# MarbleHE/ABC

Hardware: AMD Instinct MI355X
Metric: homomorphic mul+relin/sec, CKKS N=2^14 (higher is better)
Workload: dtype u64 (transforms: exact integer arithmetic in f64); 1 GPU; CKKS N=16384, 4 data limbs {50,40,40,40} + special 50-bit prime, ct x ct multiply + relinearize; total_batch=8192, batch_rank0=8192

## Files before the change

### abc_amd/csrc/abc_context.hip

```cpp
#include <cstdlib>
#include <cstring>
#include <mutex>

#include "../../include/abc_hip.h"
#include <dlfcn.h>

#include "abc_context.hpp"
#include "abc_host_math.hpp"

namespace abc {

static thread_local std::string g_err;
void set_error(const std::string &msg) { g_err = msg; }

static bool env_on(const char *name) {
  const char *e = std::getenv(name);
  return e && !(e[0] == '0' && e[1] == 0);
}
void read_switches(abc_hip_ctx *c) {
  abc_hip_ctx::Switches s;
  s.no_fused = env_on("ABC_HIP_NO_FUSED");
  s.no_split = env_on("ABC_HIP_NO_SPLIT");
  s.no_split4 = env_on("ABC_HIP_NO_SPLIT4");
  s.no_isplit = env_on("ABC_HIP_NO_ISPLIT");
  s.no_gsplit = env_on("ABC_HIP_NO_GSPLIT");
  s.no_bsplit = env_on("ABC_HIP_NO_BSPLIT");
  s.no_mixed = env_on("ABC_HIP_NO_MIXED");
  s.no_pack = env_on("ABC_HIP_NO_PACK");
  s.no_key_twin = env_on("ABC_HIP_NO_KEY_TWIN");
  s.no_bmul = env_on("ABC_HIP_NO_BMUL");
  s.no_special8x2 = env_on("ABC_HIP_NO_SPECIAL8X2");
  s.no_bmul_mid = env_on("ABC_HIP_NO_BMUL_MID");
  s.no_finish_lds = env_on("ABC_HIP_NO_FINISH_LDS");
  s.no_iks = env_on("ABC_HIP_NO_IKS");
  s.no_bmul_r6 = env_on("ABC_HIP_NO_BMUL_R6");
  s.no_lean_front = env_on("ABC_HIP_NO_LEAN_FRONT");
  s.no_tensor_intt = env_on("ABC_HIP_NO_TENSOR_INTT");
  s.no_galois_fusion = env_on("ABC_HIP_NO_GALOIS_FUSION");
  if (const char *e = std::getenv("ABC_HIP_CHUNK")) s.chunk = (size_t)std::atol(e);
  if (const char *e = std::getenv("ABC_HIP_FEW_LIMBS")) s.few_limbs = (size_t)std::atol(e);
  if (const char *e = std::getenv("ABC_HIP_LEAN_LIMIT")) s.lean_limit = (size_t)std::atol(e);
  if (const char *e = std::getenv("ABC_HIP_PASS0_TARGET_LIMIT")) s.pass0_target_limit = (size_t)std::atol(e);
  if (const char *e = std::getenv("ABC_HIP_BFV_SCRATCH_MB")) s.bfv_scratch_mb = (size_t)std::atol(e);
  if (const char *e = std::getenv("ABC_HIP_LANE_OFFSET_US")) s.lane_offset_us = (unsigned)std::atoi(e);
  if (const char *e = std::getenv("ABC_HIP_LANES")) {
    s.lanes = std::atoi(e);
    if (s.lanes < 1) s.lanes = 1;
    if (s.lanes > abc_hip_ctx::kMaxLanes) s.lanes = abc_hip_ctx::kMaxLanes;
  }
  c->sw = s;
}

static bool capturing(abc_hip_ctx *c) {
  hipStreamCaptureStatus st = hipStreamCaptureStatusNone;
  if (hipStreamIsCapturing(c->stream, &st) != hipSuccess) return false;
  return st != hipStreamCaptureStatusNone;
// ... 1091 lines not shown
```

### abc_amd/csrc/abc_context.hpp

```cpp
#pragma once

#include <hip/hip_runtime.h>

#include <map>
#include <mutex>
#include <unordered_map>
#include <string>
#include <vector>

#include "abc_modarith.hpp"
#include "abc_ntt.hpp"

namespace abc {

constexpr int kMaxLimbs = 16;

struct LimbMap {
  int id[kMaxLimbs + 1];
};

struct DevConst {
  u64 inv_special[kMaxLimbs], inv_special_s[kMaxLimbs];
  u64 inv_qlast[kMaxLimbs][kMaxLimbs], inv_qlast_s[kMaxLimbs][kMaxLimbs];
  u64 special_mod_q[kMaxLimbs], special_mod_q_s[kMaxLimbs];
// ... 73 lines not shown
}

struct abc_hip_ctx {
  int scheme = 0, logn = 0, n = 0, K = 0, L = 0, device = 0;
  std::vector<uint64_t> primes;
  uint64_t t = 0;
  hipStream_t stream = nullptr;
  hipStream_t own_stream = nullptr;
  hipEvent_t ev0 = nullptr, ev1 = nullptr;
  static constexpr int kMaxLanes = 4;
  hipStream_t lane[kMaxLanes] = {nullptr, nullptr, nullptr, nullptr};
  hipEvent_t lane_fork = nullptr, lane_join[kMaxLanes] = {nullptr, nullptr, nullptr, nullptr};
  std::vector<abc::Mod> h_mods;
  std::vector<uint64_t> mod_values;
  int nB = 0, nBsk = 0;
  abc::DevCtx dc{};
  abc::DevConst h_cst{};
  abc::Mod *d_mods = nullptr;
  uint64_t *d_tw = nullptr;
  double *d_ftw = nullptr;
  bool cache_alloc = false;
  std::mutex alloc_mu;
  size_t cached_bytes = 0, cache_cap = (size_t)8 << 30;
  std::unordered_map<size_t, std::vector<void *>> free_blocks;
  std::unordered_map<void *, size_t> block_size;
  bool capture_active = false;
  std::unordered_map<void *, std::vector<void *>> pin;
  std::unordered_map<void *, bool> parked;
  std::unordered_map<size_t, std::vector<void *>> cap_free;
  std::unordered_map<void *, bool> cap_born;
  bool behz_fp = false;
  bool use_fp = true;
  struct Switches {
    bool no_fused = false, no_split = false, no_split4 = false, no_isplit = false, no_gsplit = false, no_lean_front = false, no_bsplit = false, no_mixed = false, no_pack = false, no_key_twin = false, no_special8x2 = false, no_bmul = false, no_bmul_mid = false, no_finish_lds = false, no_iks = false, no_bmul_r6 = false, no_tensor_intt = false;
    bool no_galois_fusion = false;
    size_t chunk = 0, few_limbs = 48, lean_limit = 96, bfv_scratch_mb = 0, pass0_target_limit = 128;
    int lanes = 2;
    unsigned lane_offset_us = 0;
  } sw;
  abc::DevConst *d_cst = nullptr;
  abc::DevConstFp *d_cstf = nullptr;
  uint32_t *d_slot_map = nullptr;
  void *d_ckks_codec = nullptr;
  uint64_t *d_sk = nullptr, *d_pk = nullptr, *d_relin = nullptr;
  std::map<uint32_t, uint64_t *> d_galois;
  std::unordered_map<const uint64_t *, double *> key_twins;
  std::unordered_map<const uint64_t *, uint64_t *> key_shoups;
  std::vector<uint32_t> galois_order;
  void *ws = nullptr;
  size_t ws_bytes = 0;
  void *aux[3] = {nullptr, nullptr, nullptr};
  size_t aux_bytes[3] = {0, 0, 0};
  size_t limb_words() const { return (size_t)n; }
  size_t key_words() const { return (size_t)L * 2 * K * n; }
};

namespace abc {

void set_error(const std::string &msg);
#define ABC_HIP_CHECK(expr)                                                                         \
  do {                                                                                              \
    hipError_t e_ = (expr);                                                                         \
    if (e_ != hipSuccess) {                                                                         \
      abc::set_error(std::string(#expr) + ": " + hipGetErrorString(e_));                            \
      return 1;                                                                                     \
    }                                                                                               \
  } while (0)
// ... 107 lines not shown
```

### abc_amd/csrc/abc_kernels_fused.hip

```cpp
#include <type_traits>

#include "abc_context.hpp"
#include "abc_host_math.hpp"

namespace abc {

static inline unsigned stream_grid(size_t items, int block) {
  size_t g = (items + block - 1) / block;
  const size_t cap = 256 * 8 * 4;
  return (unsigned)(g < cap ? (g ? g : 1) : cap);
}

template <int LB>
__global__ __launch_bounds__((1 << LB) / 16) void k_fused_tensor_intt(DevCtx c, const u64 *__restrict__ a,
                                                                      const u64 *__restrict__ b, u64 *__restrict__ c01,
                                                                      u64 *__restrict__ c2coef, u64 *__restrict__ c2ntt, int nl) {
  __shared__ u64 lds[lds_words(LB)];
  const int j = blockIdx.x % nl;
  const size_t ct = blockIdx.x / nl;
  const size_t N = (size_t)1 << LB, pw = (size_t)nl * N;
  const Mod m = c.mods[j];
  const NttTable t = ntt_table(c, j);
  const u64 *__restrict__ a0 = a + ct * 2 * pw + j * N, *__restrict__ a1 = a0 + pw;
  const u64 *__restrict__ b0 = b + ct * 2 * pw + j * N, *__restrict__ b1 = b0 + pw;
// ... 788 lines not shown
    r.x = fp_to_canon(fp_mul_lazy(s1[0] - u1.x, inv, inv_q, q) + d1[0], q, qinv);
    r.y = fp_to_canon(fp_mul_lazy(s1[1] - u1.y, inv, inv_q, q) + d1[1], q, qinv);
    *reinterpret_cast<u64x2 *>(out + ((ct * 2 + 1) * nl + I) * N + base + e) = r;
  }
}

template <int MODE, bool GAL>
static void launch_split3_main(hipStream_t st, abc_hip_ctx *c, size_t cc, int nl, const double *part, const double *tpart, const u64 *opa,
                               const u64 *opb, size_t opa_stride, size_t opb_stride, int add_c1, const u64 *key, u64 *out, u32 gelt) {
  const dim3 grid((unsigned)(cc * nl * 16)), block(64 * (nl + 1));
  const size_t lds = (size_t)((nl + 1) * lds_words(10)) * 8;
#define ABC_TM3(NLV)                                                                                                                 \
  hipLaunchKernelGGL((k_split3_main_fp<MODE, GAL, NLV>), grid, block, lds, st, c->dc, part, tpart, opa, opb, opa_stride, opb_stride, \
                     add_c1, key, out, nl, gelt)
  switch (nl) {
    case 1: ABC_TM3(1); break;
    case 2: ABC_TM3(2); break;
    case 3: ABC_TM3(3); break;
    case 4: ABC_TM3(4); break;
    default: ABC_TM3(0); break;
  }
#undef ABC_TM3
}


template <int MODE, int NL>
struct PairOps {
  u64x2 k0[NL], k1[NL];
  u64x2 a0, a1, b0, b1;
  u64 xs[2], d0s[2], d1s[2];
};

template <int MODE, bool GAL, int NL>
__global__ __launch_bounds__(512, NL <= 4 ? 4 : 2) void k_split4_main_fp(DevCtx c, const double *__restrict__ part,
                                                                   const double *__restrict__ tpart, const u64 *__restrict__ opa,
                                                                   const u64 *__restrict__ opb, size_t opa_stride, size_t opb_stride,
                                                                   int add_c1, const u64 *__restrict__ key, u64 *__restrict__ out, u32 gelt,
                                                                   u32 imap, int ni, int pack, const double *__restrict__ keyf) {
  extern __shared__ double dyn[];
  static_assert(NL + 1 <= 8, "one wavefront per limb, eight wavefronts");
  constexpr int nl = NL, NT = 512, PER = 2;
  const int W = __builtin_amdgcn_readfirstlane((int)(threadIdx.x >> 6));
  const int lane = threadIdx.x & 63;
  const int blk = blockIdx.x & 15;
  const int I = (int)((imap >> (4 * ((blockIdx.x >> 4) % (unsigned)ni))) & 15u);
  const size_t ct = (size_t)((blockIdx.x >> 4) / (unsigned)ni);
  const size_t N = (size_t)c.n, base = (size_t)blk << 10;
  const Mod m = mod_at(c, I);
  const FpTable t = fp_table(c, I);
  const double q = m.qd, qinv = m.qinv;
  f64x2 *ltw = reinterpret_cast<f64x2 *>(dyn + (nl + 1) * lds_words(10));
  const size_t pw = (size_t)nl * N;
  const ABC_CONST_AS DevConst *cst = (const ABC_CONST_AS DevConst *)c.cst;
  const double inv = cst->inv_special_c[I], inv_q = cst->inv_special_cq[I];

  f64x2 twv[PER];
  block_twiddles_fetch<10, f64x2, PER>(t.tw, 4, blk, (int)threadIdx.x, NT, twv);
  const bool has_limb = W <= nl;
  const int Wc = has_limb ? W : 0;
  const double *__restrict__ src = (Wc < nl - 1) ? part + ((ct * (nl + 1) + I) * nl + (Wc < I ? Wc : Wc + 1)) * (size_t)c.ps + base
                                                 : tpart + ((ct * 2 + (Wc - (nl - 1))) * nl + I) * (size_t)c.ps + base;
  const int pk = pack ? pack_kind(m.bits) : 0;
  u64x2 raw[8];
  if (has_limb) {
    if (pk == 0) {
#pragma unroll
      for (int k = 0; k < 8; k++) raw[k] = *reinterpret_cast<const u64x2 *>(src + (k << 7) + 2 * lane);
    } else if (pk == 1) {
#pragma unroll
      for (int k = 0; k < 8; k++) raw[k] = pack_load_pair<1>(src - base, N, base + (k << 7) + 2 * lane);
    } else {
#pragma unroll
      for (int k = 0; k < 8; k++) raw[k] = pack_load_pair<2>(src - base, N, base + (k << 7) + 2 * lane);
    }
  }
  auto load_pair = [&](int e, PairOps<MODE, NL> &o) {
    const u64 *kw = keyf ? reinterpret_cast<const u64 *>(keyf) : key;
#pragma unroll
    for (int Jx = 0; Jx < NL; Jx++) {
      o.k0[Jx] = *reinterpret_cast<const u64x2 *>(kw + (((size_t)Jx * 2 + 0) * c.K + I) * N + base + e);
      o.k1[Jx] = *reinterpret_cast<const u64x2 *>(kw + (((size_t)Jx * 2 + 1) * c.K + I) * N + base + e);
    }
    if (MODE == 0) {
      const u64 *pa = opa + ct * 2 * pw + (size_t)I * N + base + e, *pb = opb + ct * 2 * pw + (size_t)I * N + base + e;
      o.a0 = *reinterpret_cast<const u64x2 *>(pa); o.a1 = *reinterpret_cast<const u64x2 *>(pa + pw);
      o.b0 = *reinterpret_cast<const u64x2 *>(pb); o.b1 = *reinterpret_cast<const u64x2 *>(pb + pw);
    } else {
      const u64 *xl = opa + ct * opa_stride + (size_t)I * N;
#pragma unroll
      for (int k = 0; k < 2; k++) {
        const u32 si = galois_ntt_src<GAL>((u32)(base + e + k), gelt, c.logn);
        o.xs[k] = xl[si];
        o.d0s[k] = o.d1s[k] = 0;
        if (opb) {
          const u64 *ad = opb + ct * opb_stride + (size_t)I * N;
          o.d0s[k] = ad[si];
          if (add_c1) o.d1s[k] = ad[pw + si];
        }
      }
    }
  };
  PairOps<MODE, NL> ops;
  load_pair(2 * (int)threadIdx.x, ops);

  block_twiddles_store<10, f64x2, PER>(ltw, (int)threadIdx.x, NT, twv);
  __syncthreads();
  if (has_limb) {
    double *buf = dyn + W * lds_words(10);
    double xin[16];
    if (pk == 0) {
#pragma unroll
      for (int k = 0; k < 8; k++) {
        xin[k] = __longlong_as_double((long long)raw[k].x);
        xin[8 + k] = __longlong_as_double((long long)raw[k].y);
      }
    } else if (pk == 1) {
#pragma unroll
      for (int k = 0; k < 8; k++) pack_decode_pair<1>(raw[k], xin[k], xin[8 + k]);
    } else {
#pragma unroll
      for (int k = 0; k < 8; k++) pack_decode_pair<2>(raw[k], xin[k], xin[8 + k]);
    }
    if (m.bits >= 49) {
#pragma unroll
      for (int r = 0; r < 16; r++) xin[r] = fp_centre(xin[r], q, qinv);
    }
    ntt_fwd_tail1024_pairs<FpTail>(buf, xin, [&](int, int i, double v) { buf[lds_pad(i)] = v; }, t, m, 4, blk, lane, ltw);
  }
  __syncthreads();
  const double *tt0 = dyn + (nl - 1) * lds_words(10), *tt1 = dyn + nl * lds_words(10);
  auto compute_pair = [&](int e, const PairOps<MODE, NL> &o, auto twin) {
    constexpr bool TW = decltype(twin)::value;
    auto kd = [](u64 w) { return TW ? __longlong_as_double((long long)w) : fp_from_u64(w); };
    double s0[2] = {0.0, 0.0}, s1[2] = {0.0, 0.0}, d0[2] = {0.0, 0.0}, d1[2] = {0.0, 0.0};
#pragma unroll
    for (int Jx = 0; Jx < NL; Jx++) {
      double x[2];
      if (Jx == I) {
        if (MODE == 0) {
          const double x0[2] = {fp_from_u64(o.a0.x), fp_from_u64(o.a0.y)}, x1[2] = {fp_from_u64(o.a1.x), fp_from_u64(o.a1.y)};
          const double y0[2] = {fp_from_u64(o.b0.x), fp_from_u64(o.b0.y)}, y1[2] = {fp_from_u64(o.b1.x), fp_from_u64(o.b1.y)};
#pragma unroll
          for (int k = 0; k < 2; k++) {
            x[k] = fp_mulmod(x1[k], y1[k], q, qinv);
            d0[k] = fp_mulmod(x0[k], y0[k], q, qinv);
            d1[k] = fp_mulmod(x0[k], y1[k], q, qinv) + fp_mulmod(x1[k], y0[k], q, qinv);
          }
        } else {
#pragma unroll
          for (int k = 0; k < 2; k++) {
            x[k] = fp_from_u64(o.xs[k]);
            d0[k] = fp_from_u64(o.d0s[k]);
            d1[k] = fp_from_u64(o.d1s[k]);
          }
        }
      } else {
        const int w = Jx < I ? Jx : Jx - 1;
        const f64x2 v = *reinterpret_cast<const f64x2 *>(dyn + w * lds_words(10) + lds_pad(e));
        x[0] = v.x;
        x[1] = v.y;
      }
      s0[0] += fp_mulmod(x[0], kd(o.k0[Jx].x), q, qinv);
      s0[1] += fp_mulmod(x[1], kd(o.k0[Jx].y), q, qinv);
      s1[0] += fp_mulmod(x[0], kd(o.k1[Jx].x), q, qinv);
      s1[1] += fp_mulmod(x[1], kd(o.k1[Jx].y), q, qinv);
      if (Jx == 7) {
#pragma unroll
        for (int k = 0; k < 2; k++) {
          s0[k] = fp_centre(s0[k], q, qinv);
          s1[k] = fp_centre(s1[k], q, qinv);
        }
      }
    }
    const f64x2 u0 = *reinterpret_cast<const f64x2 *>(tt0 + lds_pad(e)), u1 = *reinterpret_cast<const f64x2 *>(tt1 + lds_pad(e));
    u64x2 r;
    r.x = fp_to_canon(fp_mul_lazy(s0[0] - u0.x, inv, inv_q, q) + d0[0], q, qinv);
    r.y = fp_to_canon(fp_mul_lazy(s0[1] - u0.y, inv, inv_q, q) + d0[1], q, qinv);
    *reinterpret_cast<u64x2 *>(out + ((ct * 2 + 0) * nl + I) * N + base + e) = r;
    r.x = fp_to_canon(fp_mul_lazy(s1[0] - u1.x, inv, inv_q, q) + d1[0], q, qinv);
    r.y = fp_to_canon(fp_mul_lazy(s1[1] - u1.y, inv, inv_q, q) + d1[1], q, qinv);
    *reinterpret_cast<u64x2 *>(out + ((ct * 2 + 1) * nl + I) * N + base + e) = r;
  };
  if (keyf) compute_pair(2 * (int)threadIdx.x, ops, std::true_type{});
  else compute_pair(2 * (int)threadIdx.x, ops, std::false_type{});
}

template <int MODE, bool GAL>
static bool launch_split4_main(hipStream_t st, abc_hip_ctx *c, size_t cc, int nl, const double *part, const double *tpart, const u64 *opa,
                               const u64 *opb, size_t opa_stride, size_t opb_stride, int add_c1, const u64 *key, u64 *out, u32 gelt,
                               u32 imap = 0x76543210u, int ni = -1, int pack = 0) {
  if (nl < 1 || nl > 7) return false;
  if (ni < 0) ni = nl;
  if (ni == 0) return true;
  const dim3 grid((unsigned)(cc * ni * 16)), block(512);
  const size_t lds = (size_t)((nl + 1) * lds_words(10)) * 8 + 1024 * 16;
#define ABC_TM4(NLV)                                                                                                                 \
  hipLaunchKernelGGL((k_split4_main_fp<MODE, GAL, NLV>), grid, block, lds, st, c->dc, part, tpart, opa, opb, opa_stride, opb_stride, \
                     add_c1, key, out, gelt, imap, ni, pack, keyf)
  const double *keyf = key_twin_lookup(c, key);
  switch (nl) {
    case 1: ABC_TM4(1); break;
    case 2: ABC_TM4(2); break;
    case 3: ABC_TM4(3); break;
    case 4: ABC_TM4(4); break;
    case 5: ABC_TM4(5); break;
    case 6: ABC_TM4(6); break;
    default: ABC_TM4(7); break;
  }
#undef ABC_TM4
  return true;
}
bool split4_main_subset(hipStream_t st, abc_hip_ctx *c, size_t cc, int nl, int mode, const double *part, const double *tpart, const u64 *opa,
                        const u64 *opb, size_t opa_stride, size_t opb_stride, int add_c1, const u64 *key, u64 *out, u32 gelt, u32 imap,
                        int ni) {
  if (mode == 0) return launch_split4_main<0, false>(st, c, cc, nl, part, tpart, opa, opb, opa_stride, opb_stride, add_c1, key, out, gelt, imap, ni);
  if (gelt) return launch_split4_main<1, true>(st, c, cc, nl, part, tpart, opa, opb, opa_stride, opb_stride, add_c1, key, out, gelt, imap, ni);
  return launch_split4_main<1, false>(st, c, cc, nl, part, tpart, opa, opb, opa_stride, opb_stride, add_c1, key, out, gelt, imap, ni);
}


template <int MODE, bool GAL>
static void launch_split3(hipStream_t st, abc_hip_ctx *c, const FusedScratch &s, size_t cc, int nl, const u64 *opa, const u64 *opb,
                          size_t opa_stride, size_t opb_stride, int add_c1, const u64 *key, u64 *out, u32 gelt, int pack) {
  launch_split_special(st, c, cc, nl, (const double *)s.dec, key, (double *)s.tsp);
  hipLaunchKernelGGL(k_split3_pass_fp<14>, dim3((unsigned)(cc * 2 * 4)), dim3(256), 0, st, c->dc, (const double *)s.tsp, (double *)s.ksacc,
                     nl, pack);
  if (!c->sw.no_split4 && nl <= 5 && launch_split4_main<MODE, GAL>(st, c, cc, nl, (const double *)s.dec, (const double *)s.ksacc, opa, opb,
                                                        opa_stride, opb_stride, add_c1, key, out, gelt, 0x76543210u, -1, pack))
    return;
  launch_split3_main<MODE, GAL>(st, c, cc, nl, (const double *)s.dec, (const double *)s.ksacc, opa, opb, opa_stride, opb_stride, add_c1,
                                key, out, gelt);
}

static inline int pack_half_done(const abc_hip_ctx *c, int nl) {
  return (!c->sw.no_pack && !c->sw.no_split4 && nl >= 1 && nl <= 5) ? 1 : 0;
}
static inline bool all_fp(const abc_hip_ctx *c) {
  bool fp = c->use_fp;
  for (int j = 0; j < c->K; j++) fp = fp && fp_ok(c->h_mods[j].bits);
  return fp;
}
static inline bool needs_guard(const abc_hip_ctx *c) {
  bool guard = false;
  for (int j = 0; j < c->K; j++) guard = guard || !unguarded_ok(c->h_mods[j].bits);
  return guard;
}

template <int LB>
static int keyswitch_stage(abc_hip_ctx *c, hipStream_t st, const FusedScratch &s, const u64 *coef, size_t coef_stride, const u64 *ntt,
                           size_t ntt_stride, const u64 *key, const u64 *addend, size_t addend_stride, bool add_c1, u64 *out, int nl,
                           size_t cc, int dec_ready = 0 ) {
  const size_t N = (size_t)1 << LB;
  const dim3 block((1 << LB) / 16);
  const bool ckks = (c->scheme == 2);
  const bool guard = needs_guard(c);
  const unsigned g2a = (unsigned)(cc * (nl + 1) * nl);
  const unsigned g3 = (unsigned)(cc * 2 * nl);
  if (all_fp(c)) {
    if (!dec_ready)
// ... 330 lines not shown
```

### abc_amd/csrc/abc_ntt.hpp

```cpp
#pragma once

#include "abc_modarith.hpp"

namespace abc {

__device__ __forceinline__ int lds_pad(int i) { return i + ((i >> 6) << 2); }
constexpr int lds_words(int lb) { return (1 << lb) + ((1 << lb) >> 6) * 4; }

struct NttTable {
  const u64x2 *tw;
  const u64x2 *itw;
};
struct alignas(16) f64x2 {
  double x, y;
};
#define ABC_CONST_AS __attribute__((address_space(4)))
struct FpTable {
  const ABC_CONST_AS f64x2 *tw, *itw;
};
__device__ __forceinline__ f64x2 tw_load(const ABC_CONST_AS f64x2 *p) {
  f64x2 r;
  r.x = p->x;
  r.y = p->y;
  return r;
// ... 115 lines not shown
    if (PASS > 0 && k.red) centre16(x, k);
  }
  template <int PASS> __device__ __forceinline__ static void inv_begin(E (&x)[16], const K &k) {
    if (PASS > 0 || k.red) centre16(x, k);
  }
};

struct FpTail : FpArith {
  template <int PASS> __device__ __forceinline__ static void fwd_begin(E (&x)[16], const K &k) {
    if (PASS == 2 && k.red && k.q >= 562949953421312.0) centre16(x, k);
  }
};

template <class A, int LB, int S, int R>
__device__ __forceinline__ void fwd_pass(typename A::E (&x)[16], const int (&hi)[16 >> R], const typename A::Table &t,
                                         const typename A::K &kk, int S0, int b) {
  constexpr int NG = 16 >> R;
#pragma unroll
  for (int u = 0; u < R; u++) {
    const int half = 1 << (R - 1 - u);
#pragma unroll
    for (int g = 0; g < NG; g++) {
      int base = (1 << (S0 + S + u)) + (b << (S + u)) + (hi[g] << u);
#pragma unroll
      for (int k = 0; k < (1 << R); k++) {
        if (k & half) continue;
        int idx = base + (k >> (R - u));
        A::fwd(x[g * (1 << R) + k], x[g * (1 << R) + (k | half)], tw_load(t.tw + idx), kk);
      }
    }
  }
}

template <class A, int LB, int S, int R>
__device__ __forceinline__ void fwd_pass_lds(typename A::E (&x)[16], const int (&hi)[16 >> R], const typename A::TW *ltw,
                                             const typename A::K &kk) {
  constexpr int NG = 16 >> R;
#pragma unroll
  for (int u = 0; u < R; u++) {
    const int half = 1 << (R - 1 - u);
#pragma unroll
    for (int g = 0; g < NG; g++) {
      int base = (1 << (S + u)) + (hi[g] << u);
#pragma unroll
      for (int k = 0; k < (1 << R); k++) {
        if (k & half) continue;
        int idx = base + (k >> (R - u));
        A::fwd(x[g * (1 << R) + k], x[g * (1 << R) + (k | half)], ltw[idx], kk);
      }
    }
  }
}
template <int LB, class TW, int PER>
__device__ __forceinline__ void block_twiddles_fetch(const ABC_CONST_AS TW *tw, int S0, int b, int tid, int nthreads, TW (&v)[PER]) {
#pragma unroll
  for (int r = 0; r < PER; r++) {
    int mm = tid + r * nthreads;
    if (mm < 1) mm = 1;
    if (mm > (1 << LB) - 1) mm = (1 << LB) - 1;
    const int sl = 31 - __builtin_clz(mm);
    v[r] = tw_load(tw + (((1 << S0) + b) << sl) + (mm - (1 << sl)));
  }
}
template <int LB, class TW, int PER>
__device__ __forceinline__ void block_twiddles_store(TW *ltw, int tid, int nthreads, const TW (&v)[PER]) {
#pragma unroll
  for (int r = 0; r < PER; r++) {
    const int mm = tid + r * nthreads;
    if (mm >= 1 && mm < (1 << LB)) ltw[mm] = v[r];
  }
}

template <class A, int LB, int S, int R>
__device__ __forceinline__ void inv_pass(typename A::E (&x)[16], const int (&hi)[16 >> R], const typename A::Table &t,
                                         const typename A::K &kk, int S0, int b) {
  constexpr int NG = 16 >> R;
#pragma unroll
  for (int u = R - 1; u >= 0; u--) {
    const int half = 1 << (R - 1 - u);
#pragma unroll
    for (int g = 0; g < NG; g++) {
      int base = (1 << (S0 + S + u)) + (b << (S + u)) + (hi[g] << u);
#pragma unroll
      for (int k = 0; k < (1 << R); k++) {
        if (k & half) continue;
        int idx = base + (k >> (R - u));
        A::inv(x[g * (1 << R) + k], x[g * (1 << R) + (k | half)], tw_load(t.itw + idx), kk);
      }
    }
  }
}

template <class A, int LB, int S, int R>
__device__ __forceinline__ void inv_pass_lds(typename A::E (&x)[16], const int (&hi)[16 >> R], const typename A::TW *ltw,
// ... 153 lines not shown
    P::groups(tid, hi, lo);
    lds_load<LB, S, R>(lds, x, hi, lo);
    A::template fwd_begin<2>(x, kk);
    if constexpr (LTW && !P::UNIFORM) fwd_pass_lds<A, LB, S, R>(x, hi, ltw, kk);
    else fwd_pass<A, LB, S, R>(x, hi, t, kk, S0, b);
    if constexpr (SC::R3 == 0) {
#pragma unroll
      for (int g = 0; g < P::NG; g++)
#pragma unroll
        for (int k = 0; k < (1 << R); k++) store(g * (1 << R) + k, P::elem(hi[g], lo[g], k), x[g * (1 << R) + k]);
      return;
    } else {
      lds_store<LB, S, R>(lds, x, hi, lo);
    }
  }
  if constexpr (SC::R3 != 0) {
    wave_sync();
    constexpr int S = SC::R0 + SC::R1 + SC::R2, R = SC::R3;
    using P = PassIdx<LB, S, R>;
    int hi[P::NG], lo[P::NG];
    P::groups(tid, hi, lo);
    lds_load<LB, S, R>(lds, x, hi, lo);
    A::template fwd_begin<3>(x, kk);
    if constexpr (LTW && !P::UNIFORM) fwd_pass_lds<A, LB, S, R>(x, hi, ltw, kk);
    else fwd_pass<A, LB, S, R>(x, hi, t, kk, S0, b);
#pragma unroll
    for (int g = 0; g < P::NG; g++)
#pragma unroll
      for (int k = 0; k < (1 << R); k++) store(g * (1 << R) + k, P::elem(hi[g], lo[g], k), x[g * (1 << R) + k]);
  }
}


template <class A, class Store>
__device__ __forceinline__ void ntt_fwd_tail1024_pairs(typename A::E *lds, typename A::E (&x)[16], Store store,
                                                       const typename A::Table &t, const Mod &m, int S0, int b, int lane,
                                                       const typename A::TW *ltw) {
  constexpr int LB = 10;
  const typename A::K kk = A::consts(m);
  {
    const int hi[2] = {0, 0};
    fwd_pass<A, LB, 0, 3>(x, hi, t, kk, S0, b);
#pragma unroll
    for (int k = 0; k < 8; k++) {
      typename A::E *p = lds + lds_pad((k << 7) + 2 * lane);
      p[0] = x[k];
      p[1] = x[8 + k];
    }
  }
  wave_sync();
  {
    using P = PassIdx<LB, 3, 4>;
    int hi[P::NG], lo[P::NG];
    P::groups(lane, hi, lo);
    lds_load<LB, 3, 4>(lds, x, hi, lo);
    A::template fwd_begin<1>(x, kk);
    fwd_pass_lds<A, LB, 3, 4>(x, hi, ltw, kk);
    lds_store<LB, 3, 4>(lds, x, hi, lo);
  }
  wave_sync();
  {
    using P = PassIdx<LB, 7, 3>;
    int hi[P::NG], lo[P::NG];
    P::groups(lane, hi, lo);
    lds_load<LB, 7, 3>(lds, x, hi, lo);
    A::template fwd_begin<2>(x, kk);
    fwd_pass_lds<A, LB, 7, 3>(x, hi, ltw, kk);
#pragma unroll
    for (int g = 0; g < P::NG; g++)
#pragma unroll
// ... 102 lines not shown
```

Baseline: 409,300 mul+relin/s.

## Add leaner split5 keyswitch main kernel with halved LDS twiddle table

Adds a k_split5_main_fp kernel, used by default for nl<=4, that stores only the twiddle value in LDS and recomputes the Shoup companion (tw*qinv) on the fly. This halves the twiddle table footprint so that three workgroups fit per CU. It also reuses the twiddle LDS region as the buffer for the own-limb operand product, and it lets waves with no limb load their operands before the barrier. The occupancy gain comes at the cost of one extra multiply per butterfly and a different load/sync ordering. The old k_split4 logic is refactored into a shared SplitPair helper.

```diff
diff --git a/abc_amd/csrc/abc_context.hip b/abc_amd/csrc/abc_context.hip
--- a/abc_amd/csrc/abc_context.hip
+++ b/abc_amd/csrc/abc_context.hip
@@ -22,6 +22,7 @@
   s.no_fused = env_on("ABC_HIP_NO_FUSED");
   s.no_split = env_on("ABC_HIP_NO_SPLIT");
   s.no_split4 = env_on("ABC_HIP_NO_SPLIT4");
+  s.no_split5 = env_on("ABC_HIP_NO_SPLIT5");
   s.no_isplit = env_on("ABC_HIP_NO_ISPLIT");
   s.no_gsplit = env_on("ABC_HIP_NO_GSPLIT");
   s.no_bsplit = env_on("ABC_HIP_NO_BSPLIT");
diff --git a/abc_amd/csrc/abc_context.hpp b/abc_amd/csrc/abc_context.hpp
--- a/abc_amd/csrc/abc_context.hpp
+++ b/abc_amd/csrc/abc_context.hpp
@@ -129,7 +129,7 @@
   bool behz_fp = false;
   bool use_fp = true;
   struct Switches {
-    bool no_fused = false, no_split = false, no_split4 = false, no_isplit = false, no_gsplit = false, no_lean_front = false, no_bsplit = false, no_mixed = false, no_pack = false, no_key_twin = false, no_special8x2 = false, no_bmul = false, no_bmul_mid = false, no_finish_lds = false, no_iks = false, no_bmul_r6 = false, no_tensor_intt = false;
+    bool no_fused = false, no_split = false, no_split4 = false, no_split5 = false, no_isplit = false, no_gsplit = false, no_lean_front = false, no_bsplit = false, no_mixed = false, no_pack = false, no_key_twin = false, no_special8x2 = false, no_bmul = false, no_bmul_mid = false, no_finish_lds = false, no_iks = false, no_bmul_r6 = false, no_tensor_intt = false;
     bool no_galois_fusion = false;
     size_t chunk = 0, few_limbs = 48, lean_limit = 96, bfv_scratch_mb = 0, pass0_target_limit = 128;
     int lanes = 2;
diff --git a/abc_amd/csrc/abc_kernels_fused.hip b/abc_amd/csrc/abc_kernels_fused.hip
--- a/abc_amd/csrc/abc_kernels_fused.hip
+++ b/abc_amd/csrc/abc_kernels_fused.hip
@@ -844,6 +844,213 @@
 };
 
 template <int MODE, bool GAL, int NL>
+struct SplitPair {
+  const DevCtx &c;
+  const double *dyn;
+  const u64 *opa, *opb;
+  size_t opa_stride, opb_stride;
+  int add_c1;
+  const u64 *key;
+  u64 *out;
+  const double *keyf;
+  u32 gelt;
+  int I;
+  size_t ct, N, base, pw;
+  double q, qinv, inv, inv_q;
+
+  __device__ __forceinline__ void load(int e, PairOps<MODE, NL> &o) const {
+    const u64 *kw = keyf ? reinterpret_cast<const u64 *>(keyf) : key;
+#pragma unroll
+    for (int Jx = 0; Jx < NL; Jx++) {
+      o.k0[Jx] = *reinterpret_cast<const u64x2 *>(kw + (((size_t)Jx * 2 + 0) * c.K + I) * N + base + e);
+      o.k1[Jx] = *reinterpret_cast<const u64x2 *>(kw + (((size_t)Jx * 2 + 1) * c.K + I) * N + base + e);
+    }
+    if (MODE == 0) {
+      const u64 *pa = opa + ct * 2 * pw + (size_t)I * N + base + e, *pb = opb + ct * 2 * pw + (size_t)I * N + base + e;
+      o.a0 = *reinterpret_cast<const u64x2 *>(pa); o.a1 = *reinterpret_cast<const u64x2 *>(pa + pw);
+      o.b0 = *reinterpret_cast<const u64x2 *>(pb); o.b1 = *reinterpret_cast<const u64x2 *>(pb + pw);
+    } else {
+      const u64 *xl = opa + ct * opa_stride + (size_t)I * N;
+#pragma unroll
+      for (int k = 0; k < 2; k++) {
+        const u32 si = galois_ntt_src<GAL>((u32)(base + e + k), gelt, c.logn);
+        o.xs[k] = xl[si];
+        o.d0s[k] = o.d1s[k] = 0;
+        if (opb) {
+          const u64 *ad = opb + ct * opb_stride + (size_t)I * N;
+          o.d0s[k] = ad[si];
+          if (add_c1) o.d1s[k] = ad[pw + si];
+        }
+      }
+    }
+  }
+
+  template <bool TW>
+  __device__ __forceinline__ void compute(int e, const PairOps<MODE, NL> &o) const {
+    auto kd = [](u64 w) { return TW ? __longlong_as_double((long long)w) : fp_from_u64(w); };
+    double s0[2] = {0.0, 0.0}, s1[2] = {0.0, 0.0}, d0[2] = {0.0, 0.0}, d1[2] = {0.0, 0.0};
+#pragma unroll
+    for (int Jx = 0; Jx < NL; Jx++) {
+      double x[2];
+      if (Jx == I) {
+        if (MODE == 0) {
+          const double x0[2] = {fp_from_u64(o.a0.x), fp_from_u64(o.a0.y)}, x1[2] = {fp_from_u64(o.a1.x), fp_from_u64(o.a1.y)};
+          const double y0[2] = {fp_from_u64(o.b0.x), fp_from_u64(o.b0.y)}, y1[2] = {fp_from_u64(o.b1.x), fp_from_u64(o.b1.y)};
+#pragma unroll
+          for (int k = 0; k < 2; k++) {
+            x[k] = fp_mulmod(x1[k], y1[k], q, qinv);
+            d0[k] = fp_mulmod(x0[k], y0[k], q, qinv);
+            d1[k] = fp_mulmod(x0[k], y1[k], q, qinv) + fp_mulmod(x1[k], y0[k], q, qinv);
+          }
+        } else {
+#pragma unroll
+          for (int k = 0; k < 2; k++) {
+            x[k] = fp_from_u64(o.xs[k]);
+            d0[k] = fp_from_u64(o.d0s[k]);
+            d1[k] = fp_from_u64(o.d1s[k]);
+          }
+        }
+      } else {
+        const int w = Jx < I ? Jx : Jx - 1;
+        const f64x2 v = *reinterpret_cast<const f64x2 *>(dyn + w * lds_words(10) + lds_pad(e));
+        x[0] = v.x;
+        x[1] = v.y;
+      }
+      s0[0] += fp_mulmod(x[0], kd(o.k0[Jx].x), q, qinv);
+      s0[1] += fp_mulmod(x[1], kd(o.k0[Jx].y), q, qinv);
+      s1[0] += fp_mulmod(x[0], kd(o.k1[Jx].x), q, qinv);
+      s1[1] += fp_mulmod(x[1], kd(o.k1[Jx].y), q, qinv);
+      if (Jx == 7) {
+#pragma unroll
+        for (int k = 0; k < 2; k++) {
+          s0[k] = fp_centre(s0[k], q, qinv);
+          s1[k] = fp_centre(s1[k], q, qinv);
+        }
+      }
+    }
+    store(e, s0, s1, d0, d1);
+  }
+
+  __device__ __forceinline__ void store(int e, const double (&s0)[2], const double (&s1)[2], const double (&d0)[2],
+                                        const double (&d1)[2]) const {
+    constexpr int nl = NL;
+    const double *tt0 = dyn + (nl - 1) * lds_words(10), *tt1 = dyn + nl * lds_words(10);
+    const f64x2 u0 = *reinterpret_cast<const f64x2 *>(tt0 + lds_pad(e)), u1 = *reinterpret_cast<const f64x2 *>(tt1 + lds_pad(e));
+    u64x2 r;
+    r.x = fp_to_canon(fp_mul_lazy(s0[0] - u0.x, inv, inv_q, q) + d0[0], q, qinv);
+    r.y = fp_to_canon(fp_mul_lazy(s0[1] - u0.y, inv, inv_q, q) + d0[1], q, qinv);
+    *reinterpret_cast<u64x2 *>(out + ((ct * 2 + 0) * nl + I) * N + base + e) = r;
+    r.x = fp_to_canon(fp_mul_lazy(s1[0] - u1.x, inv, inv_q, q) + d1[0], q, qinv);
+    r.y = fp_to_canon(fp_mul_lazy(s1[1] - u1.y, inv, inv_q, q) + d1[1], q, qinv);
+    *reinterpret_cast<u64x2 *>(out + ((ct * 2 + 1) * nl + I) * N + base + e) = r;
+  }
+
+  struct LeanOps {
+    u64x2 k0[NL], k1[NL];
+    double xd[2], d0[2], d1[2];
+  };
+  __device__ __forceinline__ void load_lean(int e, LeanOps &o) const {
+    PairOps<MODE, 0> ab;
+    if (MODE == 0) {
+      const u64 *pa = opa + ct * 2 * pw + (size_t)I * N + base + e, *pb = opb + ct * 2 * pw + (size_t)I * N + base + e;
+      ab.a0 = *reinterpret_cast<const u64x2 *>(pa); ab.a1 = *reinterpret_cast<const u64x2 *>(pa + pw);
+      ab.b0 = *reinterpret_cast<const u64x2 *>(pb); ab.b1 = *reinterpret_cast<const u64x2 *>(pb + pw);
+    } else {
+      const u64 *xl = opa + ct * opa_stride + (size_t)I * N;
+#pragma unroll
+      for (int k = 0; k < 2; k++) {
+        const u32 si = galois_ntt_src<GAL>((u32)(base + e + k), gelt, c.logn);
+        ab.xs[k] = xl[si];
+        ab.d0s[k] = ab.d1s[k] = 0;
+        if (opb) {
+          const u64 *ad = opb + ct * opb_stride + (size_t)I * N;
+          ab.d0s[k] = ad[si];
+          if (add_c1) ab.d1s[k] = ad[pw + si];
+        }
+      }
+    }
+    const u64 *kw = keyf ? reinterpret_cast<const u64 *>(keyf) : key;
+#pragma unroll
+    for (int Jx = 0; Jx < NL; Jx++) {
+      o.k0[Jx] = *reinterpret_cast<const u64x2 *>(kw + (((size_t)Jx * 2 + 0) * c.K + I) * N + base + e);
+      o.k1[Jx] = *reinterpret_cast<const u64x2 *>(kw + (((size_t)Jx * 2 + 1) * c.K + I) * N + base + e);
+    }
+    if (MODE == 0) {
+      const double x0[2] = {fp_from_u64(ab.a0.x), fp_from_u64(ab.a0.y)}, x1[2] = {fp_from_u64(ab.a1.x), fp_from_u64(ab.a1.y)};
+      const double y0[2] = {fp_from_u64(ab.b0.x), fp_from_u64(ab.b0.y)}, y1[2] = {fp_from_u64(ab.b1.x), fp_from_u64(ab.b1.y)};
+#pragma unroll
+      for (int k = 0; k < 2; k++) {
+        o.xd[k] = fp_mulmod(x1[k], y1[k], q, qinv);
+        o.d0[k] = fp_mulmod(x0[k], y0[k], q, qinv);
+        o.d1[k] = fp_mulmod(x0[k], y1[k], q, qinv) + fp_mulmod(x1[k], y0[k], q, qinv);
+      }
+    } else {
+#pragma unroll
+      for (int k = 0; k < 2; k++) {
+        o.xd[k] = fp_from_u64(ab.xs[k]);
+        o.d0[k] = fp_from_u64(ab.d0s[k]);
+        o.d1[k] = fp_from_u64(ab.d1s[k]);
+      }
+    }
+#pragma unroll
+    for (int k = 0; k < 2; k++) asm volatile("" : "+v"(o.xd[k]), "+v"(o.d0[k]), "+v"(o.d1[k]));
+  }
+  template <bool TW>
+  __device__ __forceinline__ void compute_lean(int e, const LeanOps &o, double *dg) const {
+    auto kd = [](u64 w) { return TW ? __longlong_as_double((long long)w) : fp_from_u64(w); };
+    *reinterpret_cast<f64x2 *>(dg + lds_pad(e)) = f64x2{o.xd[0], o.xd[1]};
+    double s0[2] = {0.0, 0.0}, s1[2] = {0.0, 0.0};
+#pragma unroll
+    for (int Jx = 0; Jx < NL; Jx++) {
+      const double *src = Jx == I ? dg : dyn + (Jx < I ? Jx : Jx - 1) * lds_words(10);
+      const f64x2 v = *reinterpret_cast<const f64x2 *>(src + lds_pad(e));
+      const double x[2] = {v.x, v.y};
+      s0[0] += fp_mulmod(x[0], kd(o.k0[Jx].x), q, qinv);
+      s0[1] += fp_mulmod(x[1], kd(o.k0[Jx].y), q, qinv);
+      s1[0] += fp_mulmod(x[0], kd(o.k1[Jx].x), q, qinv);
+      s1[1] += fp_mulmod(x[1], kd(o.k1[Jx].y), q, qinv);
+    }
+    store(e, s0, s1, o.d0, o.d1);
+  }
+};
+
+__device__ __forceinline__ void split_limb_load(const double *src, size_t N, size_t base, int lane, int pk, u64x2 (&raw)[8]) {
+  if (pk == 0) {
+#pragma unroll
+    for (int k = 0; k < 8; k++) raw[k] = *reinterpret_cast<const u64x2 *>(src + (k << 7) + 2 * lane);
+  } else if (pk == 1) {
+#pragma unroll
+    for (int k = 0; k < 8; k++) raw[k] = pack_load_pair<1>(src - base, N, base + (k << 7) + 2 * lane);
+  } else {
+#pragma unroll
+    for (int k = 0; k < 8; k++) raw[k] = pack_load_pair<2>(src - base, N, base + (k << 7) + 2 * lane);
+  }
+}
+template <class LT>
+__device__ __forceinline__ void split_limb_tail(double *buf, const u64x2 (&raw)[8], int pk, const FpTable &t, const Mod &m, int blk,
+                                                int lane, const LT *ltw) {
+  double xin[16];
+  if (pk == 0) {
+#pragma unroll
+    for (int k = 0; k < 8; k++) {
+      xin[k] = __longlong_as_double((long long)raw[k].x);
+      xin[8 + k] = __longlong_as_double((long long)raw[k].y);
+    }
+  } else if (pk == 1) {
+#pragma unroll
+    for (int k = 0; k < 8; k++) pack_decode_pair<1>(raw[k], xin[k], xin[8 + k]);
+  } else {
+#pragma unroll
+    for (int k = 0; k < 8; k++) pack_decode_pair<2>(raw[k], xin[k], xin[8 + k]);
+  }
+  if (m.bits >= 49) {
+#pragma unroll
+    for (int r = 0; r < 16; r++) xin[r] = fp_centre(xin[r], m.qd, m.qinv);
+  }
+  ntt_fwd_tail1024_pairs<FpTail>(buf, xin, [&](int, int i, double v) { buf[lds_pad(i)] = v; }, t, m, 4, blk, lane, ltw);
+}
+
+template <int MODE, bool GAL, int NL>
 __global__ __launch_bounds__(512, NL <= 4 ? 4 : 2) void k_split4_main_fp(DevCtx c, const double *__restrict__ part,
                                                                    const double *__restrict__ tpart, const u64 *__restrict__ opa,
                                                                    const u64 *__restrict__ opb, size_t opa_stride, size_t opb_stride,
@@ -865,6 +1072,8 @@
   const size_t pw = (size_t)nl * N;
   const ABC_CONST_AS DevConst *cst = (const ABC_CONST_AS DevConst *)c.cst;
   const double inv = cst->inv_special_c[I], inv_q = cst->inv_special_cq[I];
+  const SplitPair<MODE, GAL, NL> sp{c, dyn, opa, opb, opa_stride, opb_stride, add_c1, key, out, keyf, gelt, I, ct, N, base, pw,
+                                    q, qinv, inv, inv_q};
 
   f64x2 twv[PER];
   block_twiddles_fetch<10, f64x2, PER>(t.tw, 4, blk, (int)threadIdx.x, NT, twv);
@@ -874,127 +1083,16 @@
                                                  : tpart + ((ct * 2 + (Wc - (nl - 1))) * nl + I) * (size_t)c.ps + base;
   const int pk = pack ? pack_kind(m.bits) : 0;
   u64x2 raw[8];
-  if (has_limb) {
-    if (pk == 0) {
-#pragma unroll
-      for (int k = 0; k < 8; k++) raw[k] = *reinterpret_cast<const u64x2 *>(src + (k << 7) + 2 * lane);
-    } else if (pk == 1) {
-#pragma unroll
-      for (int k = 0; k < 8; k++) raw[k] = pack_load_pair<1>(src - base, N, base + (k << 7) + 2 * lane);
-    } else {
-#pragma unroll
-      for (int k = 0; k < 8; k++) raw[k] = pack_load_pair<2>(src - base, N, base + (k << 7) + 2 * lane);
-    }
-  }
-  auto load_pair = [&](int e, PairOps<MODE, NL> &o) {
-    const u64 *kw = keyf ? reinterpret_cast<const u64 *>(keyf) : key;
-#pragma unroll
-    for (int Jx = 0; Jx < NL; Jx++) {
-      o.k0[Jx] = *reinterpret_cast<const u64x2 *>(kw + (((size_t)Jx * 2 + 0) * c.K + I) * N + base + e);
-      o.k1[Jx] = *reinterpret_cast<const u64x2 *>(kw + (((size_t)Jx * 2 + 1) * c.K + I) * N + base + e);
-    }
-    if (MODE == 0) {
-      const u64 *pa = opa + ct * 2 * pw + (size_t)I * N + base + e, *pb = opb + ct * 2 * pw + (size_t)I * N + base + e;
-      o.a0 = *reinterpret_cast<const u64x2 *>(pa); o.a1 = *reinterpret_cast<const u64x2 *>(pa + pw);
-      o.b0 = *reinterpret_cast<const u64x2 *>(pb); o.b1 = *reinterpret_cast<const u64x2 *>(pb + pw);
-    } else {
-      const u64 *xl = opa + ct * opa_stride + (size_t)I * N;
-#pragma unroll
-      for (int k = 0; k < 2; k++) {
-        const u32 si = galois_ntt_src<GAL>((u32)(base + e + k), gelt, c.logn);
-        o.xs[k] = xl[si];
-        o.d0s[k] = o.d1s[k] = 0;
-        if (opb) {
-          const u64 *ad = opb + ct * opb_stride + (size_t)I * N;
-          o.d0s[k] = ad[si];
-          if (add_c1) o.d1s[k] = ad[pw + si];
-        }
-      }
-    }
-  };
+  if (has_limb) split_limb_load(src, N, base, lane, pk, raw);
   PairOps<MODE, NL> ops;
-  load_pair(2 * (int)threadIdx.x, ops);
+  sp.load(2 * (int)threadIdx.x, ops);
 
   block_twiddles_store<10, f64x2, PER>(ltw, (int)threadIdx.x, NT, twv);
   __syncthreads();
-  if (has_limb) {
-    double *buf = dyn + W * lds_words(10);
-    double xin[16];
-    if (pk == 0) {
-#pragma unroll
-      for (int k = 0; k < 8; k++) {
-        xin[k] = __longlong_as_double((long long)raw[k].x);
-        xin[8 + k] = __longlong_as_double((long long)raw[k].y);
-      }
-    } else if (pk == 1) {
-#pragma unroll
-      for (int k = 0; k < 8; k++) pack_decode_pair<1>(raw[k], xin[k], xin[8 + k]);
-    } else {
-#pragma unroll
-      for (int k = 0; k < 8; k++) pack_decode_pair<2>(raw[k], xin[k], xin[8 + k]);
-    }
-    if (m.bits >= 49) {
-#pragma unroll
-      for (int r = 0; r < 16; r++) xin[r] = fp_centre(xin[r], q, qinv);
-    }
-    ntt_fwd_tail1024_pairs<FpTail>(buf, xin, [&](int, int i, double v) { buf[lds_pad(i)] = v; }, t, m, 4, blk, lane, ltw);
-  }
+  if (has_limb) split_limb_tail(dyn + W * lds_words(10), raw, pk, t, m, blk, lane, (const f64x2 *)ltw);
   __syncthreads();
-  const double *tt0 = dyn + (nl - 1) * lds_words(10), *tt1 = dyn + nl * lds_words(10);
-  auto compute_pair = [&](int e, const PairOps<MODE, NL> &o, auto twin) {
-    constexpr bool TW = decltype(twin)::value;
-    auto kd = [](u64 w) { return TW ? __longlong_as_double((long long)w) : fp_from_u64(w); };
-    double s0[2] = {0.0, 0.0}, s1[2] = {0.0, 0.0}, d0[2] = {0.0, 0.0}, d1[2] = {0.0, 0.0};
-#pragma unroll
-    for (int Jx = 0; Jx < NL; Jx++) {
-      double x[2];
-      if (Jx == I) {
-        if (MODE == 0) {
-          const double x0[2] = {fp_from_u64(o.a0.x), fp_from_u64(o.a0.y)}, x1[2] = {fp_from_u64(o.a1.x), fp_from_u64(o.a1.y)};
-          const double y0[2] = {fp_from_u64(o.b0.x), fp_from_u64(o.b0.y)}, y1[2] = {fp_from_u64(o.b1.x), fp_from_u64(o.b1.y)};
-#pragma unroll
-          for (int k = 0; k < 2; k++) {
-            x[k] = fp_mulmod(x1[k], y1[k], q, qinv);
-            d0[k] = fp_mulmod(x0[k], y0[k], q, qinv);
-            d1[k] = fp_mulmod(x0[k], y1[k], q, qinv) + fp_mulmod(x1[k], y0[k], q, qinv);
-          }
-        } else {
-#pragma unroll
-          for (int k = 0; k < 2; k++) {
-            x[k] = fp_from_u64(o.xs[k]);
-            d0[k] = fp_from_u64(o.d0s[k]);
-            d1[k] = fp_from_u64(o.d1s[k]);
-          }
-        }
-      } else {
-        const int w = Jx < I ? Jx : Jx - 1;
-        const f64x2 v = *reinterpret_cast<const f64x2 *>(dyn + w * lds_words(10) + lds_pad(e));
-        x[0] = v.x;
-        x[1] = v.y;
-      }
-      s0[0] += fp_mulmod(x[0], kd(o.k0[Jx].x), q, qinv);
-      s0[1] += fp_mulmod(x[1], kd(o.k0[Jx].y), q, qinv);
-      s1[0] += fp_mulmod(x[0], kd(o.k1[Jx].x), q, qinv);
-      s1[1] += fp_mulmod(x[1], kd(o.k1[Jx].y), q, qinv);
-      if (Jx == 7) {
-#pragma unroll
-        for (int k = 0; k < 2; k++) {
-          s0[k] = fp_centre(s0[k], q, qinv);
-          s1[k] = fp_centre(s1[k], q, qinv);
-        }
-      }
-    }
-    const f64x2 u0 = *reinterpret_cast<const f64x2 *>(tt0 + lds_pad(e)), u1 = *reinterpret_cast<const f64x2 *>(tt1 + lds_pad(e));
-    u64x2 r;
-    r.x = fp_to_canon(fp_mul_lazy(s0[0] - u0.x, inv, inv_q, q) + d0[0], q, qinv);
-    r.y = fp_to_canon(fp_mul_lazy(s0[1] - u0.y, inv, inv_q, q) + d0[1], q, qinv);
-    *reinterpret_cast<u64x2 *>(out + ((ct * 2 + 0) * nl + I) * N + base + e) = r;
-    r.x = fp_to_canon(fp_mul_lazy(s1[0] - u1.x, inv, inv_q, q) + d1[0], q, qinv);
-    r.y = fp_to_canon(fp_mul_lazy(s1[1] - u1.y, inv, inv_q, q) + d1[1], q, qinv);
-    *reinterpret_cast<u64x2 *>(out + ((ct * 2 + 1) * nl + I) * N + base + e) = r;
-  };
-  if (keyf) compute_pair(2 * (int)threadIdx.x, ops, std::true_type{});
-  else compute_pair(2 * (int)threadIdx.x, ops, std::false_type{});
+  if (keyf) sp.template compute<true>(2 * (int)threadIdx.x, ops);
+  else sp.template compute<false>(2 * (int)threadIdx.x, ops);
 }
 
 template <int MODE, bool GAL>
@@ -1031,12 +1129,86 @@
 }
 
 
+template <int MODE, bool GAL, int NL>
+__global__ __launch_bounds__(512, 6) void k_split5_main_fp(DevCtx c, const double *__restrict__ part, const double *__restrict__ tpart,
+                                                           const u64 *__restrict__ opa, const u64 *__restrict__ opb, size_t opa_stride,
+                                                           size_t opb_stride, int add_c1, const u64 *__restrict__ key,
+                                                           u64 *__restrict__ out, u32 gelt, int pack, const double *__restrict__ keyf) {
+  extern __shared__ double dyn[];
+  static_assert(NL >= 1 && NL <= 4, "nl + 1 buffers of 8.5 KiB and an 8 KiB table: three workgroups per CU up to nl = 4");
+  constexpr int nl = NL, NT = 512, PER = 2;
+  const int W = __builtin_amdgcn_readfirstlane((int)(threadIdx.x >> 6));
+  const int lane = threadIdx.x & 63;
+  const int blk = blockIdx.x & 15;
+  const int I = (int)((blockIdx.x >> 4) % (unsigned)nl);
+  const size_t ct = (size_t)((blockIdx.x >> 4) / (unsigned)nl);
+  const size_t N = (size_t)c.n, base = (size_t)blk << 10;
+  const Mod m = mod_at(c, I);
+  const FpTable t = fp_table(c, I);
+  double *ltw = dyn + (nl + 1) * lds_words(10);
+  const ABC_CONST_AS DevConst *cst = (const ABC_CONST_AS DevConst *)c.cst;
+  const SplitPair<MODE, GAL, NL> sp{c, dyn, opa, opb, opa_stride, opb_stride, add_c1, key, out, keyf, gelt, I, ct, N, base,
+                                    (size_t)nl * N, m.qd, m.qinv, cst->inv_special_c[I], cst->inv_special_cq[I]};
+  const int e = 2 * (int)threadIdx.x;
+
+  double twv[PER];
+  block_twiddles_fetch_w<10, PER>(t.tw, 4, blk, (int)threadIdx.x, NT, twv);
+  const int pk = pack ? pack_kind(m.bits) : 0;
+  typename SplitPair<MODE, GAL, NL>::LeanOps ops;
+  auto finish = [&]() {
+    if (keyf) sp.template compute_lean<true>(e, ops, ltw);
+    else sp.template compute_lean<false>(e, ops, ltw);
+  };
+  if (W <= nl) {
+    const double *__restrict__ src = (W < nl - 1) ? part + ((ct * (nl + 1) + I) * nl + (W < I ? W : W + 1)) * (size_t)c.ps + base
+                                                  : tpart + ((ct * 2 + (W - (nl - 1))) * nl + I) * (size_t)c.ps + base;
+    u64x2 raw[8];
+    split_limb_load(src, N, base, lane, pk, raw);
+    block_twiddles_store<10, double, PER>(ltw, (int)threadIdx.x, NT, twv);
+    __syncthreads();
+    split_limb_tail(dyn + W * lds_words(10), raw, pk, t, m, blk, lane, (const double *)ltw);
+    sp.load_lean(e, ops);
+    __syncthreads();
+    finish();
+  } else {
+    sp.load_lean(e, ops);
+    block_twiddles_store<10, double, PER>(ltw, (int)threadIdx.x, NT, twv);
+    __syncthreads();
+    __syncthreads();
+    finish();
+  }
+}
+
+template <int MODE, bool GAL>
+static bool launch_split5_main(hipStream_t st, abc_hip_ctx *c, size_t cc, int nl, const double *part, const double *tpart, const u64 *opa,
+                               const u64 *opb, size_t opa_stride, size_t opb_stride, int add_c1, const u64 *key, u64 *out, u32 gelt,
+                               int pack) {
+  if (nl < 1 || nl > 4) return false;
+  const dim3 grid((unsigned)(cc * nl * 16)), block(512);
+  const size_t lds = (size_t)((nl + 2) * lds_words(10)) * 8;
+  const double *keyf = key_twin_lookup(c, key);
+#define ABC_TM5(NLV)                                                                                                                 \
+  hipLaunchKernelGGL((k_split5_main_fp<MODE, GAL, NLV>), grid, block, lds, st, c->dc, part, tpart, opa, opb, opa_stride, opb_stride, \
+                     add_c1, key, out, gelt, pack, keyf)
+  switch (nl) {
+    case 1: ABC_TM5(1); break;
+    case 2: ABC_TM5(2); break;
+    case 3: ABC_TM5(3); break;
+    default: ABC_TM5(4); break;
+  }
+#undef ABC_TM5
+  return true;
+}
+
 template <int MODE, bool GAL>
 static void launch_split3(hipStream_t st, abc_hip_ctx *c, const FusedScratch &s, size_t cc, int nl, const u64 *opa, const u64 *opb,
                           size_t opa_stride, size_t opb_stride, int add_c1, const u64 *key, u64 *out, u32 gelt, int pack) {
   launch_split_special(st, c, cc, nl, (const double *)s.dec, key, (double *)s.tsp);
   hipLaunchKernelGGL(k_split3_pass_fp<14>, dim3((unsigned)(cc * 2 * 4)), dim3(256), 0, st, c->dc, (const double *)s.tsp, (double *)s.ksacc,
                      nl, pack);
+  if (!c->sw.no_split4 && !c->sw.no_split5 && launch_split5_main<MODE, GAL>(st, c, cc, nl, (const double *)s.dec, (const double *)s.ksacc,
+                                                                             opa, opb, opa_stride, opb_stride, add_c1, key, out, gelt, pack))
+    return;
   if (!c->sw.no_split4 && nl <= 5 && launch_split4_main<MODE, GAL>(st, c, cc, nl, (const double *)s.dec, (const double *)s.ksacc, opa, opb,
                                                         opa_stride, opb_stride, add_c1, key, out, gelt, 0x76543210u, -1, pack))
     return;
diff --git a/abc_amd/csrc/abc_ntt.hpp b/abc_amd/csrc/abc_ntt.hpp
--- a/abc_amd/csrc/abc_ntt.hpp
+++ b/abc_amd/csrc/abc_ntt.hpp
@@ -171,8 +171,16 @@
   }
 }
 
-template <class A, int LB, int S, int R>
-__device__ __forceinline__ void fwd_pass_lds(typename A::E (&x)[16], const int (&hi)[16 >> R], const typename A::TW *ltw,
+template <class TW, class K>
+__device__ __forceinline__ TW lds_tw(const TW *ltw, int i, const K &) { return ltw[i]; }
+__device__ __forceinline__ f64x2 lds_tw(const double *ltw, int i, const FpK &kk) {
+  f64x2 r;
+  r.x = ltw[i];
+  r.y = r.x * kk.qinv;
+  return r;
+}
+template <class A, int LB, int S, int R, class LT = typename A::TW>
+__device__ __forceinline__ void fwd_pass_lds(typename A::E (&x)[16], const int (&hi)[16 >> R], const LT *ltw,
                                              const typename A::K &kk) {
   constexpr int NG = 16 >> R;
 #pragma unroll
@@ -185,7 +193,7 @@
       for (int k = 0; k < (1 << R); k++) {
         if (k & half) continue;
         int idx = base + (k >> (R - u));
-        A::fwd(x[g * (1 << R) + k], x[g * (1 << R) + (k | half)], ltw[idx], kk);
+        A::fwd(x[g * (1 << R) + k], x[g * (1 << R) + (k | half)], lds_tw(ltw, idx, kk), kk);
       }
     }
   }
@@ -199,6 +207,18 @@
     if (mm > (1 << LB) - 1) mm = (1 << LB) - 1;
     const int sl = 31 - __builtin_clz(mm);
     v[r] = tw_load(tw + (((1 << S0) + b) << sl) + (mm - (1 << sl)));
+  }
+}
+template <int LB, int PER>
+__device__ __forceinline__ void block_twiddles_fetch_w(const ABC_CONST_AS f64x2 *tw, int S0, int b, int tid, int nthreads,
+                                                       double (&v)[PER]) {
+#pragma unroll
+  for (int r = 0; r < PER; r++) {
+    int mm = tid + r * nthreads;
+    if (mm < 1) mm = 1;
+    if (mm > (1 << LB) - 1) mm = (1 << LB) - 1;
+    const int sl = 31 - __builtin_clz(mm);
+    v[r] = tw[(((1 << S0) + b) << sl) + (mm - (1 << sl))].x;
   }
 }
 template <int LB, class TW, int PER>
@@ -418,10 +438,10 @@
 }
 
 
-template <class A, class Store>
+template <class A, class Store, class LT = typename A::TW>
 __device__ __forceinline__ void ntt_fwd_tail1024_pairs(typename A::E *lds, typename A::E (&x)[16], Store store,
                                                        const typename A::Table &t, const Mod &m, int S0, int b, int lane,
-                                                       const typename A::TW *ltw) {
+                                                       const LT *ltw ) {
   constexpr int LB = 10;
   const typename A::K kk = A::consts(m);
   {
```

Measured after the change: 412,800 mul+relin/s, median of 6. No clear change (+0.9%).
